# reinforcement-learning-kr/alpha_omok

Measured on AMD Instinct MI355X. Metric: self-play move-decisions/sec (9x9, 400 sims/move), higher is better.
Workload: dtype f32 (fp16x2-split MFMA operands, 3 products per multiply-add, f32 accumulate; inter-layer activations stored as two fp16 halves: ~22 significand bits)

## Files before the change

alpha_omok_amd/csrc/net.hip:

```cpp
#include <hip/hip_runtime.h>

#include <cmath>
#include <cstdio>
#include <cstdlib>
#include <cstring>
#include <map>
#include <type_traits>
#include <string>
#include <thread>
#include <vector>

#include "../../include/omok_hip.h"
#include "engine_types.hpp"
#include "host_handle.hpp"
#include "launchers.hpp"
#include "net_device.hpp"
#include "net_common.hpp"
#include "net_trunk_f32.hpp"
#include "net_trunk_h16.hpp"
#include "net_layer_ksplit.hpp"
#include "net_board_h16.hpp"
#include "net_small.hpp"
#include "net_w16.hpp"
#include "net_f16.hpp"
// ... 22 lines not shown
    float* conv0_w1 = nullptr;
    int nchq1 = 0;
    float *head_w3 = nullptr, *head_sc3 = nullptr, *head_sh3 = nullptr;
    float *wp_t = nullptr, *bp = nullptr, *w1_t = nullptr, *b1 = nullptr, *w2 = nullptr, *b2 = nullptr;
    int ws_boards = 0;
    float *act_x = nullptr, *act_t = nullptr, *hbuf = nullptr, *il_in = nullptr;
    float *tmp_p = nullptr, *tmp_v = nullptr;
    int* d_status = nullptr;
    bool attr_l[16][2] = {}, attr_done[16] = {}, lds_attr_done[16] = {}, attr_k[16] = {};
    int ksplit_min = 48, ksplit_max = 64, ksplit_max2 = 0;
    int rowk_min = 1, rowk_max = 47;
    bool attr_r[16] = {};
    int boardk_min = 64;
    bool attr_b[16] = {};
    long perboard_cells = 2592;
    int force_xt = 0, force_nch = 0;
    bool force_resident = false;
    ao::EventTimer timer{512};
    bool timing = false;
    int last_in_kind = 1;
    bool w16 = false;
    int products_req = 0;
    int precision_req = AO_NET_PRECISION_FP32;
    int trunk_fmt = -1;
};

template <typename T>
static int param_alloc(ao_net* n, T** out, size_t count) {
    const size_t bytes = std::max<size_t>(count * sizeof(T), 16);
    if (n->pcursor < n->pallocs.size() && n->pallocs[n->pcursor].second == bytes) {
        *out = static_cast<T*>(n->pallocs[n->pcursor++].first);
        return 0;
    }
    void* p = nullptr;
    hipError_t st = n->pool.alloc_bytes(&p, count * sizeof(T));
    if (st != hipSuccess) return n->fail(std::string("hipMalloc(") + std::to_string(bytes) + " B): " + hipGetErrorString(st));
    if (n->pcursor < n->pallocs.size()) {
        n->pool.release(n->pallocs[n->pcursor].first);
        n->pallocs[n->pcursor] = {p, bytes};
    } else {
        n->pallocs.push_back({p, bytes});
    }
    ++n->pcursor;
    *out = static_cast<T*>(p);
    return 0;
}
// ... 471 lines not shown
        a.bufA = reinterpret_cast<uint4*>(n->act_x);
        a.bufB = reinterpret_cast<uint4*>(n->act_t);
        a.nlayers = 1 + 2 * n->nb;
        a.CQ = n->CQ;
        a.COUT = n->planes;
        a.w3 = n->head_w3; a.sc3 = n->head_sc3; a.sh3 = n->head_sh3;
        a.wp_t = n->wp_t; a.bp = n->bp; a.w1_t = n->w1_t; a.b1 = n->b1; a.w2 = n->w2; a.b2 = n->b2;
        a.policy = policy;
        a.value = value;
        a.live = live; a.row_cap = row_cap;
        for (int l = 0; l < a.nlayers; ++l) {
            a.layers[l].wh = n->convh_wh[l];
            a.layers[l].wl = n->convh_wl[l];
            a.layers[l].sc = reinterpret_cast<const float4*>(n->convh_sc[l]);
            a.layers[l].sh = reinterpret_cast<const float4*>(n->conv_sh[l]);
            a.layers[l].ovf = n->d_status;
        }
        if (n->timing) n->timer.begin(s);
        if (fp16_forward(n)) {
            if (n->B > 9) return n->fail("split-fp16 trunk: board larger than 9x9");
            AO_HIP(n, ao::launch_trunk16h_f16(n->device, n->B, in_kind, groups, s, a));
        } else if (two_products(n) && n->trunk_fmt != 1) {
            if (n->B > 9) return n->fail("split-fp16 trunk: board larger than 9x9");
            AO_HIP(n, ao::launch_trunk16h_w16(n->device, n->B, in_kind, groups, s, a));
        } else
        switch (n->B) {
#define AO_BW_CASE(W)                                                                                        \
    case W: {                                                                                                \
        constexpr size_t heads_ = (static_cast<size_t>(3) * 128 + 16 * 3 * W * W + 8 * 16 * W * W + 8 * 16 * 128) * 4;  \
        constexpr size_t rows_ = static_cast<size_t>(2) * W * 4 * 2 * 1024 + 64;    \
        constexpr size_t lds_ = (rows_ > heads_) ? rows_ : heads_;                                            \
        if (!n->attr_done[W]) {                                                                                 \
            AO_HIP(n, hipFuncSetAttribute(reinterpret_cast<const void*>(&k_trunk16h<W, 4, 0>),              \
                                           hipFuncAttributeMaxDynamicSharedMemorySize, static_cast<int>(lds_))); \
            AO_HIP(n, hipFuncSetAttribute(reinterpret_cast<const void*>(&k_trunk16hb<W, 4, 0>),              \
                                           hipFuncAttributeMaxDynamicSharedMemorySize, static_cast<int>(lds_))); \
            AO_HIP(n, hipFuncSetAttribute(reinterpret_cast<const void*>(&k_trunk16h<W, 4, 1>),              \
                                           hipFuncAttributeMaxDynamicSharedMemorySize, static_cast<int>(lds_))); \
            AO_HIP(n, hipFuncSetAttribute(reinterpret_cast<const void*>(&k_trunk16hb<W, 4, 1>),              \
                                           hipFuncAttributeMaxDynamicSharedMemorySize, static_cast<int>(lds_))); \
            n->attr_done[W] = true;                                                                           \
        }                                                                                                    \
        if (n->trunk_fmt == 1) {                                                                             \
            if (in_kind == 2) hipLaunchKernelGGL((k_trunk16hb<W, 4, 1>), dim3(groups), dim3(512), lds_, s, a);    \
            else hipLaunchKernelGGL((k_trunk16h<W, 4, 1>), dim3(groups), dim3(512), lds_, s, a);                 \
        } else {                                                                                             \
            if (in_kind == 2) hipLaunchKernelGGL((k_trunk16hb<W, 4, 0>), dim3(groups), dim3(512), lds_, s, a);    \
            else hipLaunchKernelGGL((k_trunk16h<W, 4, 0>), dim3(groups), dim3(512), lds_, s, a);                 \
        }                                                                                                    \
    } break;
            AO_BW_CASE(3) AO_BW_CASE(4) AO_BW_CASE(5) AO_BW_CASE(6) AO_BW_CASE(7) AO_BW_CASE(8) AO_BW_CASE(9)
#undef AO_BW_CASE
            default: return n->fail("split-fp16 trunk: board larger than 9x9");
        }
        if (n->timing) n->timer.end(s);
        AO_HIP(n, hipGetLastError());
#ifdef AO_PROF
        if (getenv("AO_PROF_PRINT")) {
            unsigned long long h[96];
            hipStreamSynchronize(s);
            hipMemcpyFromSymbol(h, HIP_SYMBOL(ao_prof), sizeof(h));
            static const char* nm[12] = {"stage0", "slabs", "epilogue", "barrier", "last_epi+boundary", "heads", "conv1", "total",
                                         "s0:sync1", "s0:stage-issue", "s0:loads-land", "s0:sync2"};
            for (int k = 0; k < 12; ++k) {
                fprintf(stderr, "AO_PROF %-18s", nm[k]);
                for (int t = 0; t < 8; ++t) fprintf(stderr, " %9llu", h[t * 12 + k]);
                fprintf(stderr, "\n");
            }
        }
#endif
// ... 114 lines not shown
    n->nchq16 = (((inplanes + 3) / 4) + 7) & ~7;
    n->nchq1 = (((inplanes + 3) / 4) + 3) & ~3;
    n->CQ = planes / 4;
    {
        hipDeviceProp_t prop;
        if (hipGetDeviceProperties(&prop, device) == hipSuccess && prop.multiProcessorCount > 0)
            n->num_cu = prop.multiProcessorCount;
    }
    if (const char* v = getenv("AO_KSPLIT")) {
        int lo = 0, hi = 0, hi2 = 0;
        if (sscanf(v, "%d,%d,%d", &lo, &hi, &hi2) == 3) { n->ksplit_min = lo > 0 ? lo : 1 << 30; n->ksplit_max = hi; n->ksplit_max2 = hi2; }
    }
    if (const char* v = getenv("AO_PERBOARD_CELLS")) n->perboard_cells = atol(v);
    if (const char* v = getenv("AO_BOARDK")) n->boardk_min = atoi(v);
    if (const char* v = getenv("AO_ROWK")) {
        int lo = 0, hi = -1;
        if (sscanf(v, "%d,%d", &lo, &hi) == 2) { n->rowk_min = lo; n->rowk_max = hi; }
    }
    if (const char* v = getenv("AO_TRUNK_FMT")) n->trunk_fmt = atoi(v) == 1 ? 1 : 0;
    if (n->trunk_fmt < 0) n->trunk_fmt = 0;
    if (const char* v = getenv("AO_XT")) n->force_xt = atoi(v) == 4 ? 4 : (atoi(v) == 5 ? 5 : 0);
    if (const char* v = getenv("AO_NCH")) n->force_nch = atoi(v) > 0 && atoi(v) <= board ? atoi(v) : 0;
    if (const char* v = getenv("AO_FORCE_RESIDENT")) n->force_resident = atoi(v) != 0;
    return 0;
}

void ao_net_destroy(ao_net* n) {
    if (!n) return;
    hipSetDevice(n->device);
    hipDeviceSynchronize();
    n->pool.free_all();
    n->timer.destroy();
    delete n;
}

int ao_net_create(int n_block, int inplanes, int planes, int board, int device, ao_net** out) {
    if (!out) return 1;
    ao_net* n = new ao_net();
    return ao::finish_create(n, net_create_impl(n, n_block, inplanes, planes, board, device), out, ao_net_destroy);
}

int ao_net_set_mode(ao_net* n, int mode) {
    if (mode < 0 || mode > 6)
        return n->fail("mode must be 0 (auto), 1 (layer kernels), 2 (group-resident trunk), 3 (per-board), 4 (row-chunked), 5 (split-fp16 trunk) "
                       "or 6 (split-fp16 per-layer kernels for every batch size)");
    if ((mode == 5 || mode == 6) && !h16_supported(n))
// ... 296 lines not shown
             ", waves split the contraction by input block, partial tiles exchanged through LDS)";
        f = conv;
    } else if (group == 16 && mode == 5 && board_resident(n, boards)) {
        const bool one = fp16_forward(n);
        nm = std::string(one ? "k_boardh_f16<" : two_products(n) ? "k_boardh_w16<" : "k_boardh<") + bw + (in_kind == 2 ? ", 2" : ", 1") + "> (" + (in_kind == 2 ? "conv1 + " : "") + std::to_string(2 * n->nb) +
             " 3x3 convs in one launch as " + (one ? "fp16" : "split-fp16") + " MFMA 16x16x32 (" +
             (one ? "1 product: the opt-in fp16 forward, activations rounded once to fp16" : two_products(n) ? "2 products: the conv weights are fp16 numbers" : "3 products") + ", fp32 accumulate): "
             "a workgroup = one board resident in LDS through all layers, the row's cells as the MFMA N dimension, column shifts as DPP row shifts)";
        f = 2.0 * n->nb * 2.0 * n->A * 9.0 * n->planes * n->planes * boards + (in_kind == 2 ? 2.0 * n->A * 9.0 * n->C * n->planes * boards : 0.0);
    } else if (group == 16 && mode == 5 && fp16_all(n) && (layers_only(n) || !(n->B <= 9 && ((boards + 15) / 16 >= 192 || n->force_resident)))) {
        nm = "k_layer16h_f16<" + bw + "> (one 3x3 conv per launch as fp16 MFMA 16x16x32 (1 product: the opt-in fp16 forward, "
             "activations rounded once to fp16, fp32 accumulate), conv1 on " + (in_kind == 2 ? "bit planes (KIND 2)" : "float planes (KIND 1)") +
             ", 16-board groups x row chunks x column tiles)";
        f = conv;
    } else if (group == 16 && mode == 5 && (layers_only(n) || !(n->B <= 9 && ((boards + 15) / 16 >= 192 || n->force_resident)))) {
        nm = std::string(two_products(n) ? "k_layer16h_w16<" : "k_layer16h<") + bw + "> (one 3x3 conv per launch as split-fp16 MFMA 16x16x32 (" +
             (two_products(n) ? "2 products: the conv weights are fp16 numbers" : "3 products") + ", fp32 accumulate), "
             "16-board groups x row chunks x column tiles)";
        f = conv;
    } else if (group == 16 && mode == 5) {
        const bool one = fp16_forward(n);
        const bool two = !one && two_products(n) && n->trunk_fmt != 1;
        const int fmt = one ? 0 : n->trunk_fmt;
        nm = std::string(in_kind == 2 ? "k_trunk16hb" : "k_trunk16h") + (one ? "_f16<" : two ? "_w16<" : "<") + bw + ", 4, " + std::to_string(fmt) + "> (conv1 + " +
             std::to_string(2 * n->nb) + " 3x3 convs as " + (one ? "fp16" : "split-fp16") + " MFMA 16x16x32 (" +
             (one ? "1 product: the opt-in fp16 forward" : two ? "2 products: the conv weights are fp16 numbers" : "3 products") + ", fp32 accumulate) + heads, one resident "
             "launch; activations between layers as " + (one ? "one fp16" : fmt == 1 ? "fp16 high half + one low byte" : "two fp16 halves") + ")";
        f = conv1 + 2.0 * n->nb * conv;
    } else if (group == 16) {
        nm = "k_trunk16<" + bw + "> (conv1 + " + std::to_string(2 * n->nb) + " 3x3 convs, one launch, fp32 MFMA 16x16x4)";
        f = conv1 + 2.0 * n->nb * conv;
    } else {
        nm = "k_conv3x3<" + bw + "> (one 3x3 " + std::to_string(n->planes) + "->" + std::to_string(n->planes) +
             " conv, fp32 MFMA 32x32x2)";
        f = conv;
    }
    *nm_out = nm;
    *f_out = f;
}

static void copy_name(const std::string& nm, char* name, int name_cap) {
    if (name && name_cap > 0) {
        std::strncpy(name, nm.c_str(), static_cast<size_t>(name_cap) - 1);
        name[name_cap - 1] = 0;
    }
}

// ... 19 lines not shown
int ao_net_dominant_kernel(ao_net* n, int boards, char* name, int name_cap, double* flop_per_launch) {
    std::string nm;
    double f = 0.0;
    dominant_name(n, boards, n->last_in_kind, &nm, &f);
    copy_name(nm, name, name_cap);
    if (flop_per_launch) *flop_per_launch = f;
    return 0;
}

int ao_net_plan_kernel(int n_block, int inplanes, int planes, int board, int trunk_mode, int boards, int in_kind,
                       char* name, int name_cap, double* flop_per_launch) {
    if (n_block < 0 || inplanes < 1 || planes < 32 || planes % 32 || board < 3 || board > ao::kMaxBoard || boards < 1 ||
        trunk_mode < 0 || trunk_mode > 6)
        return 1;
    ao_net n;
    n.nb = n_block; n.C = inplanes; n.planes = planes; n.B = board; n.A = board * board;
    n.nchq32 = (((inplanes + 3) / 4) + 1) & ~1;
    n.nchq16 = (((inplanes + 3) / 4) + 7) & ~7;
    n.nchq1 = (((inplanes + 3) / 4) + 3) & ~3;
    n.CQ = planes / 4;
    n.mode = trunk_mode;
    if (const char* v = getenv("AO_TRUNK_FMT")) n.trunk_fmt = atoi(v) == 1 ? 1 : 0;
    if (n.trunk_fmt < 0) n.trunk_fmt = 0;
    std::string nm;
    double f = 0.0;
    dominant_name(&n, boards, in_kind, &nm, &f);
    copy_name(nm, name, name_cap);
    if (flop_per_launch) *flop_per_launch = f;
    return 0;
}

}
```

alpha_omok_amd/csrc/net_trunk_h16.hpp:

```cpp
#pragma once

#include <type_traits>

namespace ao {

struct TrunkHLayer {
    const uint4* wh;
    const uint4* wl;
    const float4* sc;
    const float4* sh;
    int* ovf;
};

struct TrunkHArgs {
    const float4* in0;
    uint4* bufA;
    uint4* bufB;
    int nlayers;
    int CQ, COUT;
    const float *w3, *sc3, *sh3, *wp_t, *bp, *w1_t, *b1, *w2, *b2;
    float* policy;
    float* value;
    const unsigned* live;
    unsigned row_cap;
// ... 66 lines not shown
__device__ __forceinline__ void row_arrive(unsigned* cnt, int lane) {
    asm volatile("s_waitcnt vmcnt(0) lgkmcnt(0)" ::: "memory");
    if (lane == 0) __hip_atomic_fetch_add(cnt, 1u, __ATOMIC_RELAXED, __HIP_MEMORY_SCOPE_WORKGROUP);
}
__device__ __forceinline__ void row_wait(unsigned* cnt, unsigned target) {
    for (;;) {
        const unsigned v = __hip_atomic_load(cnt, __ATOMIC_RELAXED, __HIP_MEMORY_SCOPE_WORKGROUP);
        if (__builtin_amdgcn_readfirstlane(v) >= target) break;
        __builtin_amdgcn_s_sleep(1);
    }
    asm volatile("" ::: "memory");
}

__host__ __device__ constexpr int kPlaneRow(int bw) { return bw * bw <= 128 ? 128 : 256; }
__host__ __device__ constexpr unsigned kPairBytes(int fmt) { return fmt == 1 ? 1536u : 2048u; }

constexpr float kLo8Scale = 0x1p-112f;
__device__ __forceinline__ float lo8_scaled(unsigned h, unsigned l) { return __uint_as_float(((h << 8) | l) << 5); }
__device__ __forceinline__ unsigned lo8_word(float vs) {
    const unsigned u = __float_as_uint(vs);
    return (u + 15u + ((u >> 5) & 1u)) >> 5;
}

template <int BW, int NC32, int NCI, int KIND, int FMT = 0, int NPROD = 3>
struct TrunkHLayerFn {
static_assert(NPROD >= 1 && NPROD <= 3, "products per multiply-add: 3 (any fp32 weights), 2 (weights on the fp16 grid), 1 (fp16 forward)");
static constexpr bool W16 = NPROD <= 2;
static constexpr bool F16 = NPROD == 1;
static_assert(!F16 || (FMT == 0 && AO_KO == 0 && !AO_CONV1_SPLIT), "the one-product form exists for the 4-byte geometry only");
static __device__ __forceinline__ void run(const void* src, uint4* dst, const TrunkHLayer& L, const bool RES, uint4* s_x,
                                           int tile, int lane, unsigned long long* prof, const bool flip,
                                           unsigned* s_cnt, const unsigned rows_before, const bool hand_next, const int par,
                                           const bool to_heads = false) {
    constexpr bool FIRST = KIND != 0;
    constexpr bool BITS = KIND == 2;
    constexpr bool HAND = FMT == 0 && AO_KO == 0;
    constexpr bool HANDED = HAND && !FIRST;
    static_assert(!HAND || NC32 >= 2, "conv1's hand-off assumes that its own row buffers lie inside the next layer's buffer 0");
    constexpr bool RES1 = BITS && HAND && !AO_CONV1_SPLIT && !AO_SPLIT_BARRIER;
    static_assert(!RES1 || (BW >= 2 && BW * BW <= 2 * BW * NC32 * 2),
                  "conv1's resident board (BW*BW high-half fragments) lies inside the two row buffers of the next layer");
    auto py = [&](int y) { return flip ? BW - 1 - y : y; };
    constexpr int A = BW * BW;
    constexpr int NT = NC32 * 2;
    constexpr int NSP = 2;
    constexpr int NFR = BW * NCI * NSP;
    constexpr int NFRO = BW * NC32 * NSP;
    constexpr int NB = NCI * 3;
    constexpr int NPR = 3;
    constexpr int PAIR = static_cast<int>(kPairBytes(FMT));
    constexpr int NPAIR = BW * NCI;
    const int kq = lane >> 4, b = lane & 15;
    const int lane16 = lane * 16;
    const int out_voff = (((tile & 1) * 2 + (kq >> 1)) * 16 + b) * 16 + (kq & 1) * 8;
    float4 sc = L.sc[tile * 4 + kq], sh = L.sh[tile * 4 + kq];
    if (FMT == 1) {
// ... 150 lines not shown
        const half2v k18 = {static_cast<_Float16>(0x1p-18f), static_cast<_Float16>(0x1p-18f)};
        const half2v m8 = {static_cast<_Float16>(-0x1p-8f), static_cast<_Float16>(-0x1p-8f)};
#pragma unroll
        for (int k = k0; k < k1; ++k) {
            const int p = tile + NT * k;
            if (p < NPAIR) {
                const uint4 hv = xb[(2 * p) * 64 + lane];
                const u32x2 lv = reinterpret_cast<const u32x2*>(xb + (2 * p + 1) * 64)[lane];
                const unsigned hw[4] = {hv.x, hv.y, hv.z, hv.w};
                unsigned ow[4];
#pragma unroll
                for (int j = 0; j < 4; ++j) {
                    const unsigned y = __builtin_amdgcn_perm(0x64646464u, lv[j >> 1], (j & 1) ? 0x04030402u : 0x04010400u);
                    const half2v c = __builtin_elementwise_fma(__builtin_bit_cast(half2v, y), k18, m8);
                    const half2v sc2 = __builtin_bit_cast(half2v, hw[j] & 0x7c007c00u);
                    ow[j] = __builtin_bit_cast(unsigned, c * sc2);
                }
                xb[(2 * p + 1) * 64 + lane] = make_uint4(ow[0], ow[1], ow[2], ow[3]);
            }
        }
    };

    const int po = ((BW & 1) || !HANDED) ? 0 : par;
    uint4* const hand2 = s_x + static_cast<size_t>(FIRST ? 1 : (BW + po) & 1) * NFRO * 64;
    uint4* const hand1 = s_x + static_cast<size_t>(FIRST ? 0 : (BW - 1 + po) & 1) * NFRO * 64;
    constexpr std::integral_constant<bool, true> kHand{};
    constexpr std::integral_constant<bool, false> kStore{};
    AO_T(t_a);
    __syncthreads();
    AO_T(t_a1);
    if (RES1) {
        constexpr int KC = (A + NT - 1) / NT;
        unsigned pb[KC];
#pragma unroll
        for (int k = 0; k < KC; ++k) {
            const int cell = tile + NT * k;
            pb[k] = cell < A ? __builtin_amdgcn_raw_buffer_load_b8(rs_src, b * kPlaneRow(BW) + cell, 0, 0) : 0u;
        }
#pragma unroll
        for (int k = 0; k < KC; ++k) {
            const int cell = tile + NT * k;
            if (cell < A) {
                half8 h;
#pragma unroll
                for (int q = 0; q < 8; ++q)
                    h[q] = (kq == 0 && ((pb[k] >> q) & 1u)) ? static_cast<_Float16>(1.0f) : static_cast<_Float16>(0.0f);
                s_x[cell * 64 + lane] = __builtin_bit_cast(uint4, h);
            }
        }
    } else if (FIRST) {
// ... 12 lines not shown
            if (f < NFR && !(AO_KO == 10 && (f & 1) && lane >= 32))
                __builtin_amdgcn_raw_ptr_buffer_load_lds(rs_src, (__attribute__((address_space(3))) void*)(s_x + f * 64), 16,
                                                         (AO_KO == 12 && (f & 1) && lane >= 32) ? lane16 - 512 : lane16,
                                                         (py(0) * NFR + f) * 1024, 0, AO_AUX_STAGE);
        }
    }
    AO_T(t_a2);
    load_w(0, wA);
    if (!HANDED) asm volatile("s_waitcnt vmcnt(0) lgkmcnt(0)" ::: "memory");
    if (FMT == 1 && !FIRST) {
        expand_pairs(s_x, 0, (NPAIR + NT - 1) / NT);
        asm volatile("s_waitcnt lgkmcnt(0)" ::: "memory");
    }
    AO_T(t_a3);
    if (!HANDED) __syncthreads();
    AO_T(t_b);
    AO_ACC(0, t_a, t_b);
    AO_ACC(8, t_a, t_a1);
    AO_ACC(9, t_a1, t_a2);
    AO_ACC(10, t_a2, t_a3);
    AO_ACC(11, t_a3, t_b);

    for (int yi = 0; yi < BW; ++yi) {
        AO_T(t_r0);
        const uint4* xs = RES1 ? s_x + static_cast<size_t>(yi) * BW * 64
                               : s_x + static_cast<size_t>((yi + po) & 1) * NFR * 64;
        auto xfrag = [&](int xi, int c, int sp) {
            return __builtin_bit_cast(half8, xs[(RES1 ? xi : (xi * NCI + c) * NSP + sp) * 64 + lane]);
        };
        uint4* xn = s_x + static_cast<size_t>((yi + 1 + po) & 1) * NFR * 64;
        const int yn = yi + 1;
        const bool stage_next = !RES1 && yn < BW && !(HANDED && yi == 0);
#pragma unroll
        for (int slab = 0; slab < NB; ++slab) {
            const int c = slab / 3, dy = slab % 3;
            half8 (&w)[2][3] = (slab & 1) ? wB : wA;
            half8 (&wn)[2][3] = (slab & 1) ? wA : wB;
            {
                const int ty = slab + 1 < NB ? yi : yi + 1, tyo = ty + 1 - (slab + 1) % 3;
                load_w(slab + 1, wn, ty < BW && tyo >= 0 && tyo < BW);
            }
            if (!stage_next) {
            } else if (dy == 1 && !AO_KO_NOSTAGE && FMT == 1 && !FIRST) {
                constexpr int K2 = (NPAIR / NT + NCI - 1) / (NCI > 1 ? NCI - 1 : 1);
                if (c > 0 && AO_KO != 11) expand_pairs(xn, (c - 1) * K2, c * K2);
                if (c + 1 < NCI) stage_pairs(yn, xn, c * K2, (c + 1) * K2);
            } else if (BITS && !AO_KO_NOSTAGE && AO_CONV1_SPLIT) {
                constexpr int KF = (NFR + NT - 1) / NT;
#pragma unroll
                for (int k = 0; k < KF; ++k) {
                    const int f = tile + NT * k;
                    if (f < NFR) {
                        if (dy == 0 && !(f & 1))
                            pbits[k] = __builtin_amdgcn_raw_buffer_load_b8(rs_src, b * kPlaneRow(BW) + yn * BW + (f >> 1), 0, 0);
                        if (dy == 2) {
// ... 41 lines not shown
                        nh = xfrag(xi + 1, c, 0);
                        nl = (RES1 || F16) ? nh : xfrag(xi + 1, c, 1);
                    }
#pragma unroll
                    for (int pr = 0; pr < NPR; ++pr) {
                        if (BITS && pr == 2) continue;
                        if (W16 && pr == 1) continue;
                        if (F16 && pr == 2) continue;
#pragma unroll
                        for (int dx = 0; dx < 3; ++dx) {
                            const int i = xi - dx + 1;
                            if (i < 0 || i >= BW) continue;
                            const half8 wv = FIRST ? wres[pr == 1 ? 1 : 0][FIRST ? dy * 3 + dx : 0] : w[pr == 1 ? 1 : 0][dx];
                            acc[2 - dy][i] = __builtin_amdgcn_mfma_f32_16x16x32_f16(wv, pr == 2 ? xl : xh, acc[2 - dy][i], 0, 0, 0);
                        }
                    }
                    xh = nh;
                    xl = nl;
                    __builtin_amdgcn_sched_barrier(0);
                }
            }
            __builtin_amdgcn_sched_barrier(0);
        }
        AO_T(t_r1);
#if AO_SPLIT_BARRIER
        row_arrive(s_cnt, lane);
#endif
        if (yi >= 1 && (!AO_KO_NOEPI || (AO_KO == 4 && yi == 1))) {
            if (HAND && hand_next && yi == BW - 1) {
                if (RES1) asm volatile("s_waitcnt lgkmcnt(0)\n\ts_barrier" ::: "memory");
                epilogue(yi - 1, kHand, hand2);
            } else {
                epilogue(yi - 1, kStore, nullptr);
            }
        }
        else if (yi >= 1 && (AO_KO == 14 || AO_KO == 15)) {
#pragma unroll
            for (int i = 0; i < BW; ++i) asm volatile("" ::"v"(acc[0][i]));
        }
#pragma unroll
        for (int i = 0; i < BW; ++i) {
            acc[0][i] = acc[1][i];
            acc[1][i] = acc[2][i];
            acc[2][i] = f32x4{0.f, 0.f, 0.f, 0.f};
        }
        AO_T(t_r2);
#if AO_SPLIT_BARRIER
        if ((yi + 1 < BW || (HAND && hand_next)) && AO_KO != 9) row_wait(s_cnt, static_cast<unsigned>(NT) * (rows_before + static_cast<unsigned>(yi) + 1u));
#else
        if (RES1) {}
        else if (AO_KO == 9) asm volatile("s_waitcnt vmcnt(0) lgkmcnt(0)" ::: "memory");
        else asm volatile("s_waitcnt vmcnt(0) lgkmcnt(0)\n\ts_barrier" ::: "memory");
#endif
        AO_T(t_r3);
        AO_ACC(1, t_r0, t_r1);
        AO_ACC(2, t_r1, t_r2);
        AO_ACC(3, t_r2, t_r3);
    }
    AO_T(t_c);
    if (!AO_KO_NOEPI || FIRST) {
        if (HAND && hand_next) epilogue(BW - 1, kHand, hand1);
        else epilogue(BW - 1, kStore, nullptr);
    }
    if (peak > (FMT == 1 ? 65504.f * kLo8Scale : 65504.f)) atomicOr(L.ovf, 1);
    asm volatile("s_waitcnt vmcnt(0)" ::: "memory");
    __syncthreads();
    __builtin_amdgcn_fence(__ATOMIC_ACQUIRE, "workgroup");
    AO_T(t_d);
    AO_ACC(4, t_c, t_d);
}
};

template <int BW, int XT, int NC32, int NCI, int KIND, int NPROD = 3>
__device__ __forceinline__ void trunk_h_layer_tile(const void* src, uint4* dst, const TrunkHLayer& L, const bool RES,
                                                   uint4* s_x, int tile, int lane, int x0, int yb, int ye) {
    static_assert(NPROD >= 1 && NPROD <= 3, "products per multiply-add: 3 (any fp32 weights), 2 (weights on the fp16 grid), 1 (fp16 forward)");
    constexpr bool W16 = NPROD <= 2;
    constexpr bool F16 = NPROD == 1;
    static_assert(!F16 || (AO_KO == 0 && !AO_CONV1_SPLIT), "the one-product form is no timing experiment");
    constexpr bool FIRST = KIND != 0;
    constexpr bool BITS = KIND == 2;
    constexpr int A = BW * BW;
    constexpr bool HALO = XT < BW;
    constexpr int NX = HALO ? XT + 2 : XT;
    constexpr int NT = NC32 * 2;
    constexpr int NSP = 2;
    constexpr int NFR = NX * NCI * NSP;
// ... 225 lines not shown
                                               a.layer, false, s_x, tile, lane, xt * XT, yb, ye);
    } else if (KIND == 1) {
        trunk_h_layer_tile<BW, XT, NC32, 1, 1, NPROD>(static_cast<const float4*>(a.src) + static_cast<size_t>(grp) * A * 8 * 16, dst, a.layer,
                                               false, s_x, tile, lane, xt * XT, yb, ye);
    } else {
        trunk_h_layer_tile<BW, XT, NC32, NC32, 0, NPROD>(static_cast<const uint4*>(a.src) + static_cast<size_t>(grp) * A * NC32 * 2 * 64, dst,
                                                      a.layer, a.res != 0, s_x, tile, lane, xt * XT, yb, ye);
    }
}

template <int BW, int XT, int NC32, int KIND>
__global__ __launch_bounds__(NC32 * 2 * 64, 1) void k_layer16h(LayerHArgs a) {
    layer16h_body<BW, XT, NC32, KIND, 3>(a);
}
template <int BW, int XT, int NC32, int KIND>
__global__ __launch_bounds__(NC32 * 2 * 64, 1) void k_layer16h_w16(LayerHArgs a) {
    layer16h_body<BW, XT, NC32, KIND, 2>(a);
}
template <int BW, int XT, int NC32, int KIND>
__global__ __launch_bounds__(NC32 * 2 * 64, 1) void k_layer16h_f16(LayerHArgs a) {
    layer16h_body<BW, XT, NC32, KIND, 1>(a);
}

template <int BW, int NC32, int INK, int FMT, int NPROD = 3>
__device__ __forceinline__ void trunk16h_body(const TrunkHArgs& a) {
    static_assert(FMT == 0 || AO_SPLIT_BARRIER == 0, "the split row barrier is implemented for the 4-byte format only");
    constexpr int A = BW * BW;
    extern __shared__ __attribute__((aligned(16))) uint4 s_x[];
    const int grp = blockIdx.x;
    if (grp >= live_groups16(a.live, a.row_cap, grp + 1)) return;
    const int lane = threadIdx.x & 63;
    const int tile = __builtin_amdgcn_readfirstlane(static_cast<int>(threadIdx.x) >> 6);
    const size_t gq = static_cast<size_t>(AO_KO == 5 ? grp % 64 : AO_KO == 6 ? grp % 128 : grp) * A * NC32 * (kPairBytes(FMT) / 16);
    uint4* bufA = a.bufA + gq;
    uint4* bufB = a.bufB + gq;
    unsigned long long prof[12] = {0, 0, 0, 0, 0, 0, 0, 0, 0, 0, 0, 0};
    unsigned long long* pp = prof;
    unsigned* s_cnt = reinterpret_cast<unsigned*>(s_x + static_cast<size_t>(2) * BW * NC32 * 2 * 64);
    if (threadIdx.x == 0) *s_cnt = 0u;
    const bool ko_fill = AO_KO == 13 || AO_KO == 15;
    AO_T(t0);
    if (INK == 2)
        TrunkHLayerFn<BW, NC32, 1, 2, FMT, NPROD>::run(reinterpret_cast<const uint8_t*>(a.in0) + static_cast<size_t>(grp) * 16 * kPlaneRow(BW), bufA,
                                      a.layers[0], false, s_x, tile, lane, pp, false, s_cnt, 0u, a.nlayers > 1, 0);
    else
        TrunkHLayerFn<BW, NC32, 1, 1, FMT, NPROD>::run(a.in0 + static_cast<size_t>(grp) * A * 8 * 16, bufA, a.layers[0], false, s_x, tile, lane, pp, false,
                                      s_cnt, 0u, a.nlayers > 1, 0);
    AO_T(t1);
    if (ko_fill) {
        __syncthreads();
        for (int f = tile; f < 2 * BW * NC32 * 2; f += NC32 * 2) s_x[f * 64 + lane] = ao_ko_fragment((grp * 4u * BW * NC32 + f) * 64u + lane, f & 1);
        __syncthreads();
    }
#ifdef AO_PROF
    for (int k = 0; k < 12; ++k) prof[k] = 0;
#endif
    static_assert(2 * BW * 16 <= NC32 * 2 * 64, "trunk_heads gives every (cell, board) of the two handed rows a thread of its own");
    const bool to_heads = FMT == 0 && AO_KO == 0 && a.nlayers > 1;
    int par = 0;
    for (int l = 1; l < a.nlayers; ++l) {
        const bool second = (l & 1) == 0;
        TrunkHLayerFn<BW, NC32, NC32, 0, FMT, NPROD>::run(second ? bufB : bufA, second ? bufA : bufB, a.layers[l], second, s_x, tile, lane, pp,
                                             (l & 1) != 0, s_cnt, static_cast<unsigned>(l) * BW, l + 1 < a.nlayers || to_heads, par,
                                             to_heads && l + 1 == a.nlayers);
        par = (par + BW - 1) & 1;
    }
    AO_T(t2);
    constexpr size_t kRowQ = static_cast<size_t>(BW) * NC32 * 2 * 64;
    if (AO_KO != 8)
        trunk_heads<BW, FMT == 1 ? 2 : NPROD == 1 ? 3 : 1>(a, reinterpret_cast<const float4*>(a.bufA), static_cast<size_t>(grp) * A, grp,
                                          to_heads ? s_x + (par ^ 1) * kRowQ : nullptr, to_heads ? s_x + par * kRowQ : nullptr);
#ifdef AO_PROF
    AO_T(t3);
    prof[5] = t3 - t2;
    prof[6] = t1 - t0;
    prof[7] = t3 - t0;
    if (grp == 5 && lane == 0)
        for (int k = 0; k < 12; ++k) ao_prof[tile * 12 + k] = prof[k];
#endif
}

template <int BW, int NC32, int FMT>
__global__ __launch_bounds__(NC32 * 2 * 64, 1) void k_trunk16h(TrunkHArgs a) {
    trunk16h_body<BW, NC32, 1, FMT>(a);
}
template <int BW, int NC32, int FMT>
__global__ __launch_bounds__(NC32 * 2 * 64, 1) void k_trunk16hb(TrunkHArgs a) {
    trunk16h_body<BW, NC32, 2, FMT>(a);
}
template <int BW, int NC32, int FMT>
__global__ __launch_bounds__(NC32 * 2 * 64, 1) void k_trunk16h_w16(TrunkHArgs a) {
    trunk16h_body<BW, NC32, 1, FMT, 2>(a);
}
template <int BW, int NC32, int FMT>
__global__ __launch_bounds__(NC32 * 2 * 64, 1) void k_trunk16hb_w16(TrunkHArgs a) {
    trunk16h_body<BW, NC32, 2, FMT, 2>(a);
}
template <int BW, int NC32, int FMT>
__global__ __launch_bounds__(NC32 * 2 * 64, 1) void k_trunk16h_f16(TrunkHArgs a) {
    trunk16h_body<BW, NC32, 1, FMT, 1>(a);
}
template <int BW, int NC32, int FMT>
__global__ __launch_bounds__(NC32 * 2 * 64, 1) void k_trunk16hb_f16(TrunkHArgs a) {
    trunk16h_body<BW, NC32, 2, FMT, 1>(a);
}

}
```

alpha_omok_amd/csrc/net_w16.hip:

```cpp
#include <hip/hip_runtime.h>

#include <cstdint>

#include "../../include/omok_hip.h"
#include "engine_types.hpp"
#include "net_device.hpp"
#include "net_common.hpp"
#include "net_trunk_f32.hpp"
#include "net_trunk_h16.hpp"
#include "net_layer_ksplit.hpp"
#include "net_board_h16.hpp"
#include "net_w16.hpp"

namespace ao {

namespace {
constexpr int kDev = 16;
bool g_attr_trunk[kDev][16][2], g_attr_layer[kDev][16][2], g_attr_board[kDev][16][2], g_attr_ksplit[kDev][16][2];

template <typename K>
hipError_t set_lds(bool* done, K kernel, size_t lds) {
    if (*done) return hipSuccess;
    const hipError_t st = hipFuncSetAttribute(reinterpret_cast<const void*>(kernel), hipFuncAttributeMaxDynamicSharedMemorySize, static_cast<int>(lds));
    if (st == hipSuccess) *done = true;
    return st;
}
}

hipError_t launch_trunk16h_w16(int device, int B, int in_kind, int groups, hipStream_t s, const TrunkHArgs& a) {
    if (device < 0 || device >= kDev) return hipErrorInvalidDevice;
    const int k = in_kind == 2 ? 1 : 0;
    switch (B) {
#define AO_BW_CASE(W)                                                                                                  \
    case W: {                                                                                                          \
        constexpr size_t heads_ = (static_cast<size_t>(3) * 128 + 16 * 3 * W * W + 8 * 16 * W * W + 8 * 16 * 128) * 4; \
        constexpr size_t rows_ = static_cast<size_t>(2) * W * 4 * 2 * 1024 + 64;                                       \
        constexpr size_t lds_ = (rows_ > heads_) ? rows_ : heads_;                                                     \
        hipError_t st = k ? set_lds(&g_attr_trunk[device][W][1], &k_trunk16hb_w16<W, 4, 0>, lds_)                      \
                          : set_lds(&g_attr_trunk[device][W][0], &k_trunk16h_w16<W, 4, 0>, lds_);                      \
        if (st != hipSuccess) return st;                                                                               \
        if (k) hipLaunchKernelGGL((k_trunk16hb_w16<W, 4, 0>), dim3(groups), dim3(512), lds_, s, a);                    \
        else hipLaunchKernelGGL((k_trunk16h_w16<W, 4, 0>), dim3(groups), dim3(512), lds_, s, a);                       \
    } break;
        AO_BW_CASE(3) AO_BW_CASE(4) AO_BW_CASE(5) AO_BW_CASE(6) AO_BW_CASE(7) AO_BW_CASE(8) AO_BW_CASE(9)
#undef AO_BW_CASE
        default: return hipErrorInvalidValue;
    }
    return hipGetLastError();
}

hipError_t launch_layer16h_w16(int device, int B, int xt, dim3 grid, hipStream_t s, const LayerHArgs& a) {
    if (device < 0 || device >= kDev) return hipErrorInvalidDevice;
#define AO_LAYERH_LAUNCH(W, XT_)                                                                                       \
    do {                                                                                                               \
        constexpr int NX_ = (XT_ < W) ? XT_ + 2 : XT_;                                                                 \
        constexpr size_t lds_ = static_cast<size_t>(2) * NX_ * 4 * 2 * 1024;                                           \
        const hipError_t st = set_lds(&g_attr_layer[device][W][XT_ == 4], &k_layer16h_w16<W, XT_, 4, 0>, lds_);        \
        if (st != hipSuccess) return st;                                                                               \
        hipLaunchKernelGGL((k_layer16h_w16<W, XT_, 4, 0>), grid, dim3(512), lds_, s, a);                               \
    } while (0)
    switch (B) {
#define AO_BW_CASE(W)                                                                                                  \
    case W: {                                                                                                          \
        if (W <= 9) AO_LAYERH_LAUNCH(W, (W <= 9 ? W : 5));                                                             \
// ... 67 lines not shown
```

alpha_omok_amd/csrc/net_w16.hpp:

```cpp
#pragma once

#include <hip/hip_runtime.h>

namespace ao {

struct TrunkHArgs;
struct LayerHArgs;
struct BoardHArgs;

hipError_t launch_trunk16h_w16(int device, int B, int in_kind, int groups, hipStream_t s, const TrunkHArgs& a);
hipError_t launch_layer16h_w16(int device, int B, int xt, dim3 grid, hipStream_t s, const LayerHArgs& a);
hipError_t launch_layer16hk_w16(int device, int B, dim3 grid, hipStream_t s, const LayerHArgs& a);
hipError_t launch_row16hk_w16(int device, int B, dim3 grid, hipStream_t s, const LayerHArgs& a);
hipError_t launch_boardh_w16(int device, int B, bool bits, dim3 grid, hipStream_t s, const BoardHArgs& a);

}
```

Measured before the change: 6544.

## Produce conv1 rows inside the first trunk layer instead of a separate phase

Adds a PRODUCE mode to the resident trunk layer. For bit-plane input, conv1's output rows are computed just ahead of when the first 3x3 layer consumes them, using an LDS copy of the plane bits and a 256-entry half8 lookup table to build the MFMA operands. This replaces the separate conv1 pass that ran before the layer loop. The intent is to interleave conv1 with the first layer's row loop and remove that pass's barriers and staging, at the cost of extra LDS and register pressure. The old path remains available via AO_TRUNK_CONV1=phase.

```diff
diff --git a/alpha_omok_amd/csrc/net.hip b/alpha_omok_amd/csrc/net.hip
--- a/alpha_omok_amd/csrc/net.hip
+++ b/alpha_omok_amd/csrc/net.hip
@@ -68,6 +68,7 @@
     bool w16 = false;
     int products_req = 0;
     int precision_req = AO_NET_PRECISION_FP32;
+    bool conv1_phase = false;
     int trunk_fmt = -1;
 };
 
@@ -585,18 +586,21 @@
             AO_HIP(n, ao::launch_trunk16h_f16(n->device, n->B, in_kind, groups, s, a));
         } else if (two_products(n) && n->trunk_fmt != 1) {
             if (n->B > 9) return n->fail("split-fp16 trunk: board larger than 9x9");
-            AO_HIP(n, ao::launch_trunk16h_w16(n->device, n->B, in_kind, groups, s, a));
+            AO_HIP(n, ao::launch_trunk16h_w16(n->device, n->B, in_kind, groups, s, a, n->conv1_phase || a.nlayers < 2));
         } else
         switch (n->B) {
 #define AO_BW_CASE(W)                                                                                        \
     case W: {                                                                                                \
         constexpr size_t heads_ = (static_cast<size_t>(3) * 128 + 16 * 3 * W * W + 8 * 16 * W * W + 8 * 16 * 128) * 4;  \
-        constexpr size_t rows_ = static_cast<size_t>(2) * W * 4 * 2 * 1024 + 64;    \
+        constexpr size_t rows_ = ao::kTrunkHRowsLds(W, 4);    \
+        static_assert(rows_ <= 160u * 1024u, "the resident trunk's LDS fits a CU");                           \
         constexpr size_t lds_ = (rows_ > heads_) ? rows_ : heads_;                                            \
         if (!n->attr_done[W]) {                                                                                 \
             AO_HIP(n, hipFuncSetAttribute(reinterpret_cast<const void*>(&k_trunk16h<W, 4, 0>),              \
                                            hipFuncAttributeMaxDynamicSharedMemorySize, static_cast<int>(lds_))); \
             AO_HIP(n, hipFuncSetAttribute(reinterpret_cast<const void*>(&k_trunk16hb<W, 4, 0>),              \
+                                           hipFuncAttributeMaxDynamicSharedMemorySize, static_cast<int>(lds_))); \
+            AO_HIP(n, hipFuncSetAttribute(reinterpret_cast<const void*>(&k_trunk16hb<W, 4, 0, 1>),           \
                                            hipFuncAttributeMaxDynamicSharedMemorySize, static_cast<int>(lds_))); \
             AO_HIP(n, hipFuncSetAttribute(reinterpret_cast<const void*>(&k_trunk16h<W, 4, 1>),              \
                                            hipFuncAttributeMaxDynamicSharedMemorySize, static_cast<int>(lds_))); \
@@ -608,7 +612,9 @@
             if (in_kind == 2) hipLaunchKernelGGL((k_trunk16hb<W, 4, 1>), dim3(groups), dim3(512), lds_, s, a);    \
             else hipLaunchKernelGGL((k_trunk16h<W, 4, 1>), dim3(groups), dim3(512), lds_, s, a);                 \
         } else {                                                                                             \
-            if (in_kind == 2) hipLaunchKernelGGL((k_trunk16hb<W, 4, 0>), dim3(groups), dim3(512), lds_, s, a);    \
+            if (in_kind == 2 && (n->conv1_phase || a.nlayers < 2))                                               \
+                hipLaunchKernelGGL((k_trunk16hb<W, 4, 0, 1>), dim3(groups), dim3(512), lds_, s, a);              \
+            else if (in_kind == 2) hipLaunchKernelGGL((k_trunk16hb<W, 4, 0>), dim3(groups), dim3(512), lds_, s, a);    \
             else hipLaunchKernelGGL((k_trunk16h<W, 4, 0>), dim3(groups), dim3(512), lds_, s, a);                 \
         }                                                                                                    \
     } break;
@@ -769,6 +775,7 @@
     if (const char* v = getenv("AO_XT")) n->force_xt = atoi(v) == 4 ? 4 : (atoi(v) == 5 ? 5 : 0);
     if (const char* v = getenv("AO_NCH")) n->force_nch = atoi(v) > 0 && atoi(v) <= board ? atoi(v) : 0;
     if (const char* v = getenv("AO_FORCE_RESIDENT")) n->force_resident = atoi(v) != 0;
+    if (const char* v = getenv("AO_TRUNK_CONV1")) n->conv1_phase = std::strcmp(v, "phase") == 0;
     return 0;
 }
 
@@ -1111,7 +1118,10 @@
         const bool one = fp16_forward(n);
         const bool two = !one && two_products(n) && n->trunk_fmt != 1;
         const int fmt = one ? 0 : n->trunk_fmt;
-        nm = std::string(in_kind == 2 ? "k_trunk16hb" : "k_trunk16h") + (one ? "_f16<" : two ? "_w16<" : "<") + bw + ", 4, " + std::to_string(fmt) + "> (conv1 + " +
+        const bool rows = ao::kTrunkConv1Rows && in_kind == 2 && !one && fmt == 0 && n->nb > 0 && !n->conv1_phase;
+        const bool phase = in_kind == 2 && !one && fmt == 0 && !rows;
+        nm = std::string(in_kind == 2 ? "k_trunk16hb" : "k_trunk16h") + (one ? "_f16<" : two ? "_w16<" : "<") + bw + ", 4, " + std::to_string(fmt) + (phase ? ", 1" : "") +
+             (rows ? "> (conv1 row by row inside the first of " : "> (conv1 + ") +
              std::to_string(2 * n->nb) + " 3x3 convs as " + (one ? "fp16" : "split-fp16") + " MFMA 16x16x32 (" +
              (one ? "1 product: the opt-in fp16 forward" : two ? "2 products: the conv weights are fp16 numbers" : "3 products") + ", fp32 accumulate) + heads, one resident "
              "launch; activations between layers as " + (one ? "one fp16" : fmt == 1 ? "fp16 high half + one low byte" : "two fp16 halves") + ")";
@@ -1177,6 +1187,7 @@
     n.mode = trunk_mode;
     if (const char* v = getenv("AO_TRUNK_FMT")) n.trunk_fmt = atoi(v) == 1 ? 1 : 0;
     if (n.trunk_fmt < 0) n.trunk_fmt = 0;
+    if (const char* v = getenv("AO_TRUNK_CONV1")) n.conv1_phase = std::strcmp(v, "phase") == 0;
     std::string nm;
     double f = 0.0;
     dominant_name(&n, boards, in_kind, &nm, &f);
diff --git a/alpha_omok_amd/csrc/net_trunk_h16.hpp b/alpha_omok_amd/csrc/net_trunk_h16.hpp
--- a/alpha_omok_amd/csrc/net_trunk_h16.hpp
+++ b/alpha_omok_amd/csrc/net_trunk_h16.hpp
@@ -112,16 +112,24 @@
     return (u + 15u + ((u >> 5) & 1u)) >> 5;
 }
 
-template <int BW, int NC32, int NCI, int KIND, int FMT = 0, int NPROD = 3>
+__host__ __device__ constexpr size_t kTrunkHCntOffset(int bw, int nc32) { return static_cast<size_t>(2) * bw * nc32 * 2 * 1024; }
+__host__ __device__ constexpr size_t kTrunkHBitsOffset(int bw, int nc32) { return kTrunkHCntOffset(bw, nc32) + 64; }
+__host__ __device__ constexpr size_t kTrunkHBitsBytes(int bw) { return static_cast<size_t>(bw) * 16 * 16; }
+__host__ __device__ constexpr size_t kTrunkHLutOffset(int bw, int nc32) { return kTrunkHBitsOffset(bw, nc32) + kTrunkHBitsBytes(bw); }
+__host__ __device__ constexpr size_t kTrunkHRowsLds(int bw, int nc32) { return kTrunkHLutOffset(bw, nc32) + 256 * 16; }
+template <int BW, int NC32, int NCI, int KIND, int FMT = 0, int NPROD = 3, bool PRODUCE = false>
 struct TrunkHLayerFn {
 static_assert(NPROD >= 1 && NPROD <= 3, "products per multiply-add: 3 (any fp32 weights), 2 (weights on the fp16 grid), 1 (fp16 forward)");
+static_assert(!PRODUCE || (KIND == 0 && FMT == 0 && NPROD >= 2 && NCI == NC32 && AO_KO == 0 && !AO_CONV1_SPLIT && !AO_SPLIT_BARRIER && BW <= 16),
+              "conv1's rows are produced inside a trunk layer of the 4-byte format, split forms, default build only");
+static_assert(!PRODUCE || (kTrunkHRowsLds(BW, NC32) <= 160u * 1024u && NC32 * 2 * 64 >= 512), "row buffers + counter + plane bytes + fragment table fit the CU's 160 KB of LDS");
 static constexpr bool W16 = NPROD <= 2;
 static constexpr bool F16 = NPROD == 1;
 static_assert(!F16 || (FMT == 0 && AO_KO == 0 && !AO_CONV1_SPLIT), "the one-product form exists for the 4-byte geometry only");
 static __device__ __forceinline__ void run(const void* src, uint4* dst, const TrunkHLayer& L, const bool RES, uint4* s_x,
                                            int tile, int lane, unsigned long long* prof, const bool flip,
                                            unsigned* s_cnt, const unsigned rows_before, const bool hand_next, const int par,
-                                           const bool to_heads = false) {
+                                           const bool to_heads = false, const void* bits = nullptr, const TrunkHLayer* P = nullptr) {
     constexpr bool FIRST = KIND != 0;
     constexpr bool BITS = KIND == 2;
     constexpr bool HAND = FMT == 0 && AO_KO == 0;
@@ -318,10 +326,110 @@
     };
 
     const int po = ((BW & 1) || !HANDED) ? 0 : par;
-    uint4* const hand2 = s_x + static_cast<size_t>(FIRST ? 1 : (BW + po) & 1) * NFRO * 64;
+    const __amdgpu_buffer_rsrc_t rs_bits = make_rsrc(bits, 16u * kPlaneRow(BW));
+    const __amdgpu_buffer_rsrc_t rs_pwh = make_rsrc(PRODUCE ? P->wh : L.wh, 9u * NT * 1024u);
+    const __amdgpu_buffer_rsrc_t rs_pwl = make_rsrc(PRODUCE ? P->wl : L.wl, 9u * NT * 1024u);
+    const uint4* const s_bits = reinterpret_cast<const uint4*>(reinterpret_cast<const char*>(s_x) + kTrunkHBitsOffset(BW, NC32));
+    const uint4* const s_lut = reinterpret_cast<const uint4*>(reinterpret_cast<const char*>(s_x) + kTrunkHLutOffset(BW, NC32));
+    const unsigned kq0 = kq == 0 ? 0xffffffffu : 0u;
+    float ppeak = 0.f;
+    auto pload = [&](int dy, half8 (&W)[2][3]) {
+#pragma unroll
+        for (int dx = 0; dx < 3; ++dx) {
+            W[0][dx] = buf_ld_h8(rs_pwh, lane16, ((dy * 3 + dx) * NT + tile) * 1024);
+            if (!W16) W[1][dx] = buf_ld_h8(rs_pwl, lane16, ((dy * 3 + dx) * NT + tile) * 1024);
+        }
+    };
+    auto produce = [&](int r, uint4* xb) {
+        const int p = py(r);
+        half8 wC[2][3];
+        auto taps = [&](int dy, half8 (&W)[2][3]) {
+            const int iy = p - 1 + dy;
+            if (iy < 0 || iy >= BW) return;
+            const uint4 pb = s_bits[iy * 16 + b];
+            const unsigned pw[4] = {pb.x & kq0, pb.y & kq0, pb.z & kq0, pb.w & kq0};
+            auto cell = [&](int xi) { return __builtin_bit_cast(half8, s_lut[(pw[xi >> 2] >> (8 * (xi & 3))) & 0xffu]); };
+            half8 xh = cell(0);
+#pragma unroll
+            for (int xi = 0; xi < BW; ++xi) {
+                half8 nh = xh;
+                if (xi + 1 < BW) nh = cell(xi + 1);
+#pragma unroll
+                for (int pr = 0; pr < 2; ++pr) {
+                    if (W16 && pr == 1) continue;
+#pragma unroll
+                    for (int dx = 0; dx < 3; ++dx) {
+                        const int i = xi - dx + 1;
+                        if (i < 0 || i >= BW) continue;
+                        acc[2][i] = __builtin_amdgcn_mfma_f32_16x16x32_f16(W[pr][dx], xh, acc[2][i], 0, 0, 0);
+                    }
+                }
+                xh = nh;
+                __builtin_amdgcn_sched_barrier(0);
+            }
+        };
+        pload(1, wC);
+        taps(0, wB);
+        __builtin_amdgcn_sched_barrier(0);
+        pload(2, wB);
+        taps(1, wC);
+        __builtin_amdgcn_sched_barrier(0);
+        taps(2, wB);
+        int pq = tile * 4 + kq;
+        asm volatile("" : "+v"(pq));
+        const float4 psc = P->sc[pq], psh = P->sh[pq];
+#pragma unroll
+        for (int i = 0; i < BW; ++i) {
+            const f32x4 c = acc[2][i];
+            const float f[4] = {fmaf(c[0], psc.x, psh.x), fmaf(c[1], psc.y, psh.y), fmaf(c[2], psc.z, psh.z), fmaf(c[3], psc.w, psh.w)};
+            ppeak = fmaxf(fmaxf(ppeak, fmaxf(f[0], f[1])), fmaxf(f[2], f[3]));
+            half4 hh, hl;
+#pragma unroll
+            for (int k = 0; k < 4; ++k) {
+                const float v = fminf(fmaxf(f[k], 0.f), 65504.f);
+                hh[k] = static_cast<_Float16>(v);
+                hl[k] = static_cast<_Float16>(v - static_cast<float>(hh[k]));
+            }
+            u32x2* hp = reinterpret_cast<u32x2*>(reinterpret_cast<char*>(xb) + (i * NC32 + (tile >> 1)) * 2048 + out_voff);
+            hp[0] = __builtin_bit_cast(u32x2, hh);
+            hp[128] = __builtin_bit_cast(u32x2, hl);
+            const int ob = ((p * BW + i) * NC32 + (tile >> 1)) * PAIR;
+            buf_st_h4(hh, rs_src, out_voff, ob);
+            buf_st_h4(hl, rs_src, out_voff, ob + 1024);
+            acc[2][i] = f32x4{0.f, 0.f, 0.f, 0.f};
+        }
+    };
+    uint4* const hand2 =s_x + static_cast<size_t>(FIRST ? 1 : (BW + po) & 1) * NFRO * 64;
     uint4* const hand1 = s_x + static_cast<size_t>(FIRST ? 0 : (BW - 1 + po) & 1) * NFRO * 64;
     constexpr std::integral_constant<bool, true> kHand{};
     constexpr std::integral_constant<bool, false> kStore{};
+    if (PRODUCE) {
+        AO_T(t_p0);
+        const int t = tile * 64 + lane;
+        if (t < 16 * BW) {
+            unsigned pbv[BW];
+#pragma unroll
+            for (int x = 0; x < BW; ++x)
+                pbv[x] = __builtin_amdgcn_raw_buffer_load_b8(rs_bits, (t & 15) * kPlaneRow(BW) + (t >> 4) * BW + x, 0, 0);
+            unsigned pw[4] = {0u, 0u, 0u, 0u};
+#pragma unroll
+            for (int x = 0; x < BW; ++x) pw[x >> 2] |= (pbv[x] & 0xffu) << (8 * (x & 3));
+            reinterpret_cast<uint4*>(reinterpret_cast<char*>(s_x) + kTrunkHBitsOffset(BW, NC32))[t] = make_uint4(pw[0], pw[1], pw[2], pw[3]);
+        }
+        if (t >= 256 && t < 512) {
+            half8 h;
+#pragma unroll
+            for (int q = 0; q < 8; ++q) h[q] = (((t - 256) >> q) & 1) ? static_cast<_Float16>(1.0f) : static_cast<_Float16>(0.0f);
+            reinterpret_cast<uint4*>(reinterpret_cast<char*>(s_x) + kTrunkHLutOffset(BW, NC32))[t - 256] = __builtin_bit_cast(uint4, h);
+        }
+        pload(0, wB);
+        __syncthreads();
+        produce(0, s_x + static_cast<size_t>(po & 1) * NFR * 64);
+        pload(0, wB);
+        produce(1, s_x + static_cast<size_t>((1 + po) & 1) * NFR * 64);
+        AO_T(t_p1);
+        AO_ACC(6, t_p0, t_p1);
+    }
     AO_T(t_a);
     __syncthreads();
     AO_T(t_a1);
@@ -380,6 +488,12 @@
     AO_ACC(11, t_a3, t_b);
 
     for (int yi = 0; yi < BW; ++yi) {
+        if (PRODUCE && yi >= 1 && yi + 1 < BW) {
+            AO_T(t_q0);
+            produce(yi + 1, s_x + static_cast<size_t>((yi + 1 + po) & 1) * NFR * 64);
+            AO_T(t_q1);
+            AO_ACC(6, t_q0, t_q1);
+        }
         AO_T(t_r0);
         const uint4* xs = RES1 ? s_x + static_cast<size_t>(yi) * BW * 64
                                : s_x + static_cast<size_t>((yi + po) & 1) * NFR * 64;
@@ -388,7 +502,7 @@
         };
         uint4* xn = s_x + static_cast<size_t>((yi + 1 + po) & 1) * NFR * 64;
         const int yn = yi + 1;
-        const bool stage_next = !RES1 && yn < BW && !(HANDED && yi == 0);
+        const bool stage_next = !RES1 && !PRODUCE && yn < BW && !(HANDED && yi == 0);
 #pragma unroll
         for (int slab = 0; slab < NB; ++slab) {
             const int c = slab / 3, dy = slab % 3;
@@ -476,6 +590,7 @@
             }
             __builtin_amdgcn_sched_barrier(0);
         }
+        if (PRODUCE && yi + 2 < BW) pload(0, wB);
         AO_T(t_r1);
 #if AO_SPLIT_BARRIER
         row_arrive(s_cnt, lane);
@@ -517,6 +632,7 @@
         else epilogue(BW - 1, kStore, nullptr);
     }
     if (peak > (FMT == 1 ? 65504.f * kLo8Scale : 65504.f)) atomicOr(L.ovf, 1);
+    if (PRODUCE && ppeak > 65504.f) atomicOr(P->ovf, 1);
     asm volatile("s_waitcnt vmcnt(0)" ::: "memory");
     __syncthreads();
     __builtin_amdgcn_fence(__ATOMIC_ACQUIRE, "workgroup");
@@ -788,9 +904,11 @@
     layer16h_body<BW, XT, NC32, KIND, 1>(a);
 }
 
-template <int BW, int NC32, int INK, int FMT, int NPROD = 3>
+constexpr bool kTrunkConv1Rows = AO_KO == 0 && !AO_CONV1_SPLIT && !AO_SPLIT_BARRIER;
+template <int BW, int NC32, int INK, int FMT, int NPROD = 3, bool C1ROWS = false>
 __device__ __forceinline__ void trunk16h_body(const TrunkHArgs& a) {
     static_assert(FMT == 0 || AO_SPLIT_BARRIER == 0, "the split row barrier is implemented for the 4-byte format only");
+    constexpr bool ROWS = C1ROWS && kTrunkConv1Rows && INK == 2 && FMT == 0 && NPROD >= 2;
     constexpr int A = BW * BW;
     extern __shared__ __attribute__((aligned(16))) uint4 s_x[];
     const int grp = blockIdx.x;
@@ -806,7 +924,17 @@
     if (threadIdx.x == 0) *s_cnt = 0u;
     const bool ko_fill = AO_KO == 13 || AO_KO == 15;
     AO_T(t0);
-    if (INK == 2)
+    int par = 0;
+    int l0 = 1;
+    static_assert(2 * BW * 16 <= NC32 * 2 * 64, "trunk_heads gives every (cell, board) of the two handed rows a thread of its own");
+    const bool to_heads = FMT == 0 && AO_KO == 0 && a.nlayers > 1;
+    if (ROWS) {
+        TrunkHLayerFn<BW, NC32, NC32, 0, FMT, NPROD, ROWS>::run(bufA, bufB, a.layers[1], false, s_x, tile, lane, pp, true, s_cnt, static_cast<unsigned>(BW),
+                                                              true, par, false, reinterpret_cast<const uint8_t*>(a.in0) + static_cast<size_t>(grp) * 16 * kPlaneRow(BW),
+                                                              &a.layers[0]);
+        par = (par + BW - 1) & 1;
+        l0 = 2;
+    } else if (INK == 2)
         TrunkHLayerFn<BW, NC32, 1, 2, FMT, NPROD>::run(reinterpret_cast<const uint8_t*>(a.in0) + static_cast<size_t>(grp) * 16 * kPlaneRow(BW), bufA,
                                       a.layers[0], false, s_x, tile, lane, pp, false, s_cnt, 0u, a.nlayers > 1, 0);
     else
@@ -819,12 +947,10 @@
         __syncthreads();
     }
 #ifdef AO_PROF
-    for (int k = 0; k < 12; ++k) prof[k] = 0;
-#endif
-    static_assert(2 * BW * 16 <= NC32 * 2 * 64, "trunk_heads gives every (cell, board) of the two handed rows a thread of its own");
-    const bool to_heads = FMT == 0 && AO_KO == 0 && a.nlayers > 1;
-    int par = 0;
-    for (int l = 1; l < a.nlayers; ++l) {
+    if (!ROWS)
+        for (int k = 0; k < 12; ++k) prof[k] = 0;
+#endif
+    for (int l = l0; l < a.nlayers; ++l) {
         const bool second = (l & 1) == 0;
         TrunkHLayerFn<BW, NC32, NC32, 0, FMT, NPROD>::run(second ? bufB : bufA, second ? bufA : bufB, a.layers[l], second, s_x, tile, lane, pp,
                                              (l & 1) != 0, s_cnt, static_cast<unsigned>(l) * BW, l + 1 < a.nlayers || to_heads, par,
@@ -839,7 +965,7 @@
 #ifdef AO_PROF
     AO_T(t3);
     prof[5] = t3 - t2;
-    prof[6] = t1 - t0;
+    if (!ROWS) prof[6] = t1 - t0;
     prof[7] = t3 - t0;
     if (grp == 5 && lane == 0)
         for (int k = 0; k < 12; ++k) ao_prof[tile * 12 + k] = prof[k];
@@ -850,17 +976,17 @@
 __global__ __launch_bounds__(NC32 * 2 * 64, 1) void k_trunk16h(TrunkHArgs a) {
     trunk16h_body<BW, NC32, 1, FMT>(a);
 }
-template <int BW, int NC32, int FMT>
+template <int BW, int NC32, int FMT, int C1PHASE = 0>
 __global__ __launch_bounds__(NC32 * 2 * 64, 1) void k_trunk16hb(TrunkHArgs a) {
-    trunk16h_body<BW, NC32, 2, FMT>(a);
+    trunk16h_body<BW, NC32, 2, FMT, 3, C1PHASE == 0>(a);
 }
 template <int BW, int NC32, int FMT>
 __global__ __launch_bounds__(NC32 * 2 * 64, 1) void k_trunk16h_w16(TrunkHArgs a) {
     trunk16h_body<BW, NC32, 1, FMT, 2>(a);
 }
-template <int BW, int NC32, int FMT>
+template <int BW, int NC32, int FMT, int C1PHASE = 0>
 __global__ __launch_bounds__(NC32 * 2 * 64, 1) void k_trunk16hb_w16(TrunkHArgs a) {
-    trunk16h_body<BW, NC32, 2, FMT, 2>(a);
+    trunk16h_body<BW, NC32, 2, FMT, 2, C1PHASE == 0>(a);
 }
 template <int BW, int NC32, int FMT>
 __global__ __launch_bounds__(NC32 * 2 * 64, 1) void k_trunk16h_f16(TrunkHArgs a) {
diff --git a/alpha_omok_amd/csrc/net_w16.hip b/alpha_omok_amd/csrc/net_w16.hip
--- a/alpha_omok_amd/csrc/net_w16.hip
+++ b/alpha_omok_amd/csrc/net_w16.hip
@@ -16,7 +16,7 @@
 
 namespace {
 constexpr int kDev = 16;
-bool g_attr_trunk[kDev][16][2], g_attr_layer[kDev][16][2], g_attr_board[kDev][16][2], g_attr_ksplit[kDev][16][2];
+bool g_attr_trunk[kDev][16][3], g_attr_layer[kDev][16][2], g_attr_board[kDev][16][2], g_attr_ksplit[kDev][16][2];
 
 template <typename K>
 hipError_t set_lds(bool* done, K kernel, size_t lds) {
@@ -27,19 +27,22 @@
 }
 }
 
-hipError_t launch_trunk16h_w16(int device, int B, int in_kind, int groups, hipStream_t s, const TrunkHArgs& a) {
+hipError_t launch_trunk16h_w16(int device, int B, int in_kind, int groups, hipStream_t s, const TrunkHArgs& a, bool conv1_phase) {
     if (device < 0 || device >= kDev) return hipErrorInvalidDevice;
-    const int k = in_kind == 2 ? 1 : 0;
+    const int k = in_kind != 2 ? 0 : conv1_phase ? 2 : 1;
     switch (B) {
 #define AO_BW_CASE(W)                                                                                                  \
     case W: {                                                                                                          \
         constexpr size_t heads_ = (static_cast<size_t>(3) * 128 + 16 * 3 * W * W + 8 * 16 * W * W + 8 * 16 * 128) * 4; \
-        constexpr size_t rows_ = static_cast<size_t>(2) * W * 4 * 2 * 1024 + 64;                                       \
+        constexpr size_t rows_ = kTrunkHRowsLds(W, 4);    \
+        static_assert(rows_ <= 160u * 1024u, "the resident trunk's LDS fits a CU");                                    \
         constexpr size_t lds_ = (rows_ > heads_) ? rows_ : heads_;                                                     \
-        hipError_t st = k ? set_lds(&g_attr_trunk[device][W][1], &k_trunk16hb_w16<W, 4, 0>, lds_)                      \
-                          : set_lds(&g_attr_trunk[device][W][0], &k_trunk16h_w16<W, 4, 0>, lds_);                      \
+        hipError_t st = k == 2 ? set_lds(&g_attr_trunk[device][W][2], &k_trunk16hb_w16<W, 4, 0, 1>, lds_)              \
+                      : k == 1 ? set_lds(&g_attr_trunk[device][W][1], &k_trunk16hb_w16<W, 4, 0>, lds_)                 \
+                               : set_lds(&g_attr_trunk[device][W][0], &k_trunk16h_w16<W, 4, 0>, lds_);                 \
         if (st != hipSuccess) return st;                                                                               \
-        if (k) hipLaunchKernelGGL((k_trunk16hb_w16<W, 4, 0>), dim3(groups), dim3(512), lds_, s, a);                    \
+        if (k == 2) hipLaunchKernelGGL((k_trunk16hb_w16<W, 4, 0, 1>), dim3(groups), dim3(512), lds_, s, a);            \
+        else if (k) hipLaunchKernelGGL((k_trunk16hb_w16<W, 4, 0>), dim3(groups), dim3(512), lds_, s, a);               \
         else hipLaunchKernelGGL((k_trunk16h_w16<W, 4, 0>), dim3(groups), dim3(512), lds_, s, a);                       \
     } break;
         AO_BW_CASE(3) AO_BW_CASE(4) AO_BW_CASE(5) AO_BW_CASE(6) AO_BW_CASE(7) AO_BW_CASE(8) AO_BW_CASE(9)
diff --git a/alpha_omok_amd/csrc/net_w16.hpp b/alpha_omok_amd/csrc/net_w16.hpp
--- a/alpha_omok_amd/csrc/net_w16.hpp
+++ b/alpha_omok_amd/csrc/net_w16.hpp
@@ -8,7 +8,7 @@
 struct LayerHArgs;
 struct BoardHArgs;
 
-hipError_t launch_trunk16h_w16(int device, int B, int in_kind, int groups, hipStream_t s, const TrunkHArgs& a);
+hipError_t launch_trunk16h_w16(int device, int B, int in_kind, int groups, hipStream_t s, const TrunkHArgs& a, bool conv1_phase);
 hipError_t launch_layer16h_w16(int device, int B, int xt, dim3 grid, hipStream_t s, const LayerHArgs& a);
 hipError_t launch_layer16hk_w16(int device, int B, dim3 grid, hipStream_t s, const LayerHArgs& a);
 hipError_t launch_row16hk_w16(int device, int B, dim3 grid, hipStream_t s, const LayerHArgs& a);
```

After: 6576, median of 6. Within noise of the previous version (+0.5%).
